# hellboywyh/pytorch-kaldi-CGS

Measured on AMD Instinct MI355X. Metric: acoustic frames/sec (train), higher is better.
Workload: dtype bf16; 1 GPU; TIMIT_baselines MLP 440-5x1024-{1928,48} (TIMIT_MLP_fmllr.cfg), batch_size_train=128, dropout 0.15, SGD body + RMSprop heads; global_batch=128, parallelism=dp1, chunk_frames_per_rank=225345

## Files before the change

### pytorch-kaldi-cgs_amd/csrc/pkc_fused.hip

```cpp
#include "pkc_common.h"

namespace pkc {
namespace fused {

constexpr int NW = 8, NT = 64 * NW;
constexpr int MR = 128;
constexpr int NC = 16;
constexpr int MT = MR / 16;

typedef __attribute__((ext_vector_type(8))) __bf16 bf8;
typedef __attribute__((ext_vector_type(4))) float f32x4;

#ifdef PKC_TRACE
constexpr int FTRACE_WG = 4096;
__device__ unsigned long long ftrace_buf[FTRACE_WG * 8];
__device__ __forceinline__ void ftrace(int i) {
  asm volatile("s_waitcnt vmcnt(0) lgkmcnt(0)" ::: "memory");
  const unsigned long long v = (i == 0 || i == 7) ? __builtin_amdgcn_s_memrealtime()
                                                  : __builtin_amdgcn_s_memtime();
  if (threadIdx.x == 0 && blockIdx.x < FTRACE_WG)
    reinterpret_cast<volatile unsigned long long*>(ftrace_buf)[blockIdx.x * 8 + i] = v;
}
#define PKC_FTR(i) ::pkc::fused::ftrace(i)
#else
#define PKC_FTR(i) do { } while (0)
#endif

__device__ __forceinline__ bf8 zero8() {
  bf8 v;
#pragma unroll
  for (int j = 0; j < 8; ++j) v[j] = (__bf16)0.f;
  return v;
}

template <bool BIN>
__device__ __forceinline__ bf8 ld8(const void* base, int64_t off) {
  if constexpr (BIN) {
    return *reinterpret_cast<const bf8*>(reinterpret_cast<const __bf16*>(base) + off);
  } else {
    const float* p = reinterpret_cast<const float*>(base) + off;
    const float4 x = *reinterpret_cast<const float4*>(p);
    const float4 y = *reinterpret_cast<const float4*>(p + 4);
    bf8 v;
    v[0] = (__bf16)x.x; v[1] = (__bf16)x.y; v[2] = (__bf16)x.z; v[3] = (__bf16)x.w;
    v[4] = (__bf16)y.x; v[5] = (__bf16)y.y; v[6] = (__bf16)y.z; v[7] = (__bf16)y.w;
    return v;
  }
}

constexpr int ROWS = MR + NC;
constexpr int IMG_BYTES = ROWS * 64;
constexpr int WAVE_BYTES = 2 * IMG_BYTES;
constexpr int STAGE_BYTES = NW * WAVE_BYTES;
constexpr int DMA_PER_STEP = ROWS * 4 / 64;

typedef __attribute__((address_space(3))) void lds_void;
typedef __attribute__((address_space(1))) const void glb_void;

__device__ __forceinline__ int img_h(int r) { return (-(r >> 2)) & 3; }

struct SlotSrc {
  int64_t off;
  bool isb;
  int k0;
};
__device__ __forceinline__ SlotSrc slot_src(int i, int lane, int ks, int M, int64_t lda, int64_t ldb,
                                            int n0) {
  const int r = 16 * i + (lane >> 2);
  const int kq = (lane & 3) ^ img_h(r);
  SlotSrc o;
  o.k0 = 32 * ks + 8 * kq;
  o.isb = r >= MR;
  o.off = o.isb ? (int64_t)(n0 + r - MR) * ldb + o.k0 : (int64_t)min(r, M - 1) * lda + o.k0;
  return o;
}

template <bool BIN>
__device__ __forceinline__ void stage_regs(char* img, const void* __restrict__ A, int64_t lda,
                                           const void* __restrict__ B, int64_t ldb, int M, int K,
                                           int n0, int ks) {
  const int lane = threadIdx.x & 63;
  const bf8 z8 = zero8();
  bf8 v[DMA_PER_STEP];
#pragma unroll
  for (int i = 0; i < DMA_PER_STEP; ++i) {
    const SlotSrc o = slot_src(i, lane, ks, M, lda, ldb, n0);
    const bool ok = o.k0 < K;
    const int64_t off = ok ? o.off : 0;
    const bf8 x = ld8<BIN>(o.isb ? B : A, off);
    v[i] = ok ? x : z8;
  }
#pragma unroll
  for (int i = 0; i < DMA_PER_STEP; ++i)
    *reinterpret_cast<bf8*>(img + 1024 * i + 16 * lane) = v[i];
}

__device__ __forceinline__ void stage_dma(char* img, const __bf16* __restrict__ A, int64_t lda,
                                          const __bf16* __restrict__ B, int64_t ldb, int M, int n0,
                                          int ks) {
  const int lane = threadIdx.x & 63;
#pragma unroll
  for (int i = 0; i < DMA_PER_STEP; ++i) {
    const SlotSrc o = slot_src(i, lane, ks, M, lda, ldb, n0);
    __builtin_amdgcn_global_load_lds((glb_void*)((o.isb ? B : A) + o.off),
                                     (lds_void*)(img + 1024 * i), 16, 0, 0);
  }
}

template <bool BIN>
__device__ __forceinline__ void strip_product(char* stage, const void* __restrict__ A, int64_t lda,
                                              const void* __restrict__ B, int64_t ldb, int M,
                                              int K, int n0, f32x4 (&acc)[MT]) {
  const int lane = threadIdx.x & 63;
  const int w = __builtin_amdgcn_readfirstlane(threadIdx.x >> 6);
  const int c = lane & 15, q = lane >> 4;
  const int nks = (K + 31) / 32;
  const int ks0 = w * nks / NW, ks1 = (w + 1) * nks / NW;
  const int nst = ks1 - ks0;
  char* mine = stage + w * WAVE_BYTES;
#pragma unroll
  for (int t = 0; t < MT; ++t) acc[t] = f32x4{0.f, 0.f, 0.f, 0.f};
  const int hq = (q ^ img_h(c)) * 16;
  const int afr = 64 * c + hq, bfr = 64 * (MR + c) + hq;
  const __bf16* Ab = reinterpret_cast<const __bf16*>(A);
  const __bf16* Bb = reinterpret_cast<const __bf16*>(B);
  auto issue = [&](int i) {
    char* img = mine + (i & 1) * IMG_BYTES;
    const int ks = ks0 + i;
    if (BIN && 32 * (ks + 1) <= K) stage_dma(img, Ab, lda, Bb, ldb, M, n0, ks);
    else stage_regs<BIN>(img, A, lda, B, ldb, M, K, n0, ks);
  };
  if (nst > 0) issue(0);
  if (nst > 1) issue(1);
  for (int i = 0; i < nst; ++i) {
    if (i + 1 < nst) asm volatile("s_waitcnt vmcnt(9)" ::: "memory");
    else asm volatile("s_waitcnt vmcnt(0)" ::: "memory");
    const char* img = mine + (i & 1) * IMG_BYTES;
    bf8 a[MT];
#pragma unroll
    for (int t = 0; t < MT; ++t) a[t] = *reinterpret_cast<const bf8*>(img + 1024 * t + afr);
    const bf8 b = *reinterpret_cast<const bf8*>(img + bfr);
    asm volatile("s_waitcnt lgkmcnt(0)" ::: "memory");
    if (i + 2 < nst) issue(i + 2);
#pragma unroll
    for (int t = 0; t < MT; ++t)
      acc[t] = __builtin_amdgcn_mfma_f32_16x16x32_bf16(a[t], b, acc[t], 0, 0, 0);
  }
}

__device__ __forceinline__ float4 strip_reduce(const f32x4 (&acc)[MT], float* red) {
  const int lane = threadIdx.x & 63, w = threadIdx.x >> 6;
  const int c = lane & 15, q = lane >> 4;
  float* mine = red + w * MR * NC;
#pragma unroll
  for (int t = 0; t < MT; ++t)
#pragma unroll
    for (int i = 0; i < 4; ++i) mine[(16 * t + 4 * q + i) * NC + c] = acc[t][i];
  __syncthreads();
  const int row = threadIdx.x >> 2, cg = threadIdx.x & 3;
  float4 z = *reinterpret_cast<const float4*>(red + row * NC + 4 * cg);
#pragma unroll
  for (int v = 1; v < NW; ++v) {
    const float4 p = *reinterpret_cast<const float4*>(red + v * MR * NC + row * NC + 4 * cg);
    z.x += p.x; z.y += p.y; z.z += p.z; z.w += p.w;
  }
  return z;
}

__device__ __forceinline__ float4 col_sum(float4 v, float4* xr) {
#pragma unroll
  for (int o = 4; o < 64; o <<= 1) {
    v.x += __shfl_xor(v.x, o, 64);
    v.y += __shfl_xor(v.y, o, 64);
    v.z += __shfl_xor(v.z, o, 64);
    v.w += __shfl_xor(v.w, o, 64);
  }
  const int lane = threadIdx.x & 63, w = threadIdx.x >> 6, cg = threadIdx.x & 3;
  if (lane < 4) xr[w * 4 + lane] = v;
  __syncthreads();
  float4 s = xr[cg];
#pragma unroll
  for (int u = 1; u < NW; ++u) {
    const float4 p = xr[u * 4 + cg];
    s.x += p.x; s.y += p.y; s.z += p.z; s.w += p.w;
  }
  return s;
}

__device__ __forceinline__ float f4g(const float4& v, int j) {
  return j == 0 ? v.x : (j == 1 ? v.y : (j == 2 ? v.z : v.w));
}
__device__ __forceinline__ void f4s(float4& v, int j, float x) {
  if (j == 0) v.x = x; else if (j == 1) v.y = x; else if (j == 2) v.z = x; else v.w = x;
}
__device__ __forceinline__ void st_h4(void* p, int64_t i, float4 v) {
  typedef __attribute__((ext_vector_type(4))) __bf16 bf16x4;
  bf16x4 h;
  h[0] = (__bf16)v.x; h[1] = (__bf16)v.y; h[2] = (__bf16)v.z; h[3] = (__bf16)v.w;
  *reinterpret_cast<bf16x4*>(reinterpret_cast<__bf16*>(p) + i) = h;
}

template <bool BIN>
__global__ __launch_bounds__(NT) void dense_gemm_fwd_kernel(const void* __restrict__ A, int64_t lda,
                                                           const void* __restrict__ W, int64_t ldw,
                                                           int K, pkc_dense_fwd_args a) {
  __shared__ __attribute__((aligned(16))) char stage[STAGE_BYTES];
  __shared__ float4 xr[2][NW * 4];
  float* red = reinterpret_cast<float*>(stage);
  static_assert(NW * MR * NC * 4 <= STAGE_BYTES, "partial strips must fit the staging LDS");
  PKC_FTR(0);
  const int n0 = blockIdx.x * NC;
  const int M = a.M;
  const int64_t N = a.N;
  const int row = threadIdx.x >> 2, cg = threadIdx.x & 3;
  const int c = n0 + 4 * cg;
  const float* dummy = a.gamma ? a.gamma : a.bias;
  const bool hb = a.bias != nullptr, bnp = a.norm != PKC_NORM_NONE && dummy != nullptr;
  const float* pd = dummy ? dummy : reinterpret_cast<const float*>(a.save_mean);
  const float4 b0 = *reinterpret_cast<const float4*>(hb ? a.bias + c : pd);
  const float4 g0 = *reinterpret_cast<const float4*>(bnp ? a.gamma + c : pd);
  const float4 be0 = *reinterpret_cast<const float4*>(bnp ? a.beta + c : pd);
  const float4 rm0 = *reinterpret_cast<const float4*>(bnp ? a.running_mean + c : pd);
  const float4 rv0 = *reinterpret_cast<const float4*>(bnp ? a.running_var + c : pd);
  const int64_t step = a.step_ctr ? *a.step_ctr : 0;
  PKC_FTR(1);
  f32x4 acc[MT];
  strip_product<BIN>(stage, A, lda, W, ldw, M, K, n0, acc);
  __syncthreads();
  PKC_FTR(2);
  float4 z = strip_reduce(acc, red);
  PKC_FTR(3);
  const bool rok = row < M;
  if (hb) z = make_float4(z.x + b0.x, z.y + b0.y, z.z + b0.z, z.w + b0.w);
  if (!rok) z = make_float4(0.f, 0.f, 0.f, 0.f);
  float4 mean = make_float4(0.f, 0.f, 0.f, 0.f), invstd = make_float4(1.f, 1.f, 1.f, 1.f);
  float4 gam = make_float4(1.f, 1.f, 1.f, 1.f), bet = make_float4(0.f, 0.f, 0.f, 0.f);
  if (a.norm == PKC_NORM_BN_TRAIN) {
    const float4 sum = col_sum(z, xr[0]);
    const float inv = 1.f / (float)M;
    mean = make_float4(sum.x * inv, sum.y * inv, sum.z * inv, sum.w * inv);
    float4 d2 = make_float4(0.f, 0.f, 0.f, 0.f);
    if (rok) {
      const float dx = z.x - mean.x, dy = z.y - mean.y, dz = z.z - mean.z, dw = z.w - mean.w;
      d2 = make_float4(dx * dx, dy * dy, dz * dz, dw * dw);
    }
    const float4 m2 = col_sum(d2, xr[1]);
    const float4 var = make_float4(m2.x * inv, m2.y * inv, m2.z * inv, m2.w * inv);
    invstd = make_float4(1.f / sqrtf(var.x + a.eps), 1.f / sqrtf(var.y + a.eps),
                         1.f / sqrtf(var.z + a.eps), 1.f / sqrtf(var.w + a.eps));
    gam = g0;
    bet = be0;
    if (row == 0) {
      *reinterpret_cast<float4*>(a.save_mean + c) = mean;
      *reinterpret_cast<float4*>(a.save_invstd + c) = invstd;
      const float cn = (float)(a.count_n > 0 ? a.count_n : M);
      float4 rm = rm0, rv = rv0;
#pragma unroll
      for (int j = 0; j < 4; ++j) {
        const float vj = f4g(var, j);
        const float unb = cn > 1.f ? vj * cn / (cn - 1.f) : vj;
        f4s(rm, j, (1.f - a.momentum) * f4g(rm, j) + a.momentum * f4g(mean, j));
        f4s(rv, j, (1.f - a.momentum) * f4g(rv, j) + a.momentum * unb);
      }
      *reinterpret_cast<float4*>(a.running_mean + c) = rm;
      *reinterpret_cast<float4*>(a.running_var + c) = rv;
    }
    PKC_FTR(4);
  } else if (a.norm == PKC_NORM_BN_EVAL) {
    mean = rm0;
    invstd = make_float4(1.f / sqrtf(rv0.x + a.eps), 1.f / sqrtf(rv0.y + a.eps),
                         1.f / sqrtf(rv0.z + a.eps), 1.f / sqrtf(rv0.w + a.eps));
    gam = g0;
    bet = be0;
  }
  if (!rok) return;
  const bool drop = a.drop_p > 0.f;
  const float scale = drop ? 1.f / (1.f - a.drop_p) : 1.f;
  const uint32_t thr = drop ? (uint32_t)((double)(1.f - a.drop_p) * 4294967296.0) : 0u;
  const uint32_t seed32 = hash_seed(a.seed, (uint64_t)a.stream_id, (uint64_t)step);
  const int64_t idx = (int64_t)row * N + c;
  float4 xh, o;
  uint32_t kw = 0;
  uchar4 kin = make_uchar4(1, 1, 1, 1);
  if (drop && a.keep_in) kin = *reinterpret_cast<const uchar4*>(a.keep_in + idx);
#pragma unroll
  for (int j = 0; j < 4; ++j) {
    const float zj = f4g(z, j);
    const float x = (a.norm == PKC_NORM_NONE) ? zj : (zj - f4g(mean, j)) * f4g(invstd, j);
    const float y = (a.norm == PKC_NORM_NONE) ? zj : x * f4g(gam, j) + f4g(bet, j);
    float v = act_fwd(a.act, y);
    if (drop) {
      uint32_t k;
      if (a.keep_in) k = j == 0 ? kin.x : (j == 1 ? kin.y : (j == 2 ? kin.z : kin.w));
      else k = hash_drop(seed32, (uint32_t)(idx + j)) < thr;
      kw |= (k ? 1u : 0u) << (8 * j);
      v = k ? v * scale : 0.f;
    }
    f4s(xh, j, x);
    f4s(o, j, v);
  }
  if (drop && a.keep_out) *reinterpret_cast<uint32_t*>(a.keep_out + idx) = kw;
  if (a.xhat) *reinterpret_cast<float4*>(a.xhat + idx) = xh;
  if (a.out) *reinterpret_cast<float4*>(a.out + idx) = o;
  if (a.out_bf16) st_h4(a.out_bf16, idx, o);
  PKC_FTR(5);
  PKC_FTR(7);
}

}
}

#ifdef PKC_TRACE
extern "C" int pkc_trace_read_fused(unsigned long long* host, int n) {
  return hipMemcpyFromSymbol(host, HIP_SYMBOL(pkc::fused::ftrace_buf), sizeof(unsigned long long) * n,
                             0, hipMemcpyDeviceToHost) == hipSuccess ? 0 : -1;
}
#endif

static bool al16(const void* p) { return (uintptr_t)p % 16 == 0; }

extern "C" int pkc_dense_gemm_fwd_ok(int prec, int M, int N, int K, const void* A, int64_t lda,
                                     const void* W, int64_t ldw) {
  using namespace pkc::fused;
  return (prec == PKC_PREC_BF16 || prec == PKC_PREC_BF16IN) && M > 0 && M <= MR && N > 0 &&
         N % NC == 0 && K > 0 && K % 8 == 0 && lda >= K && ldw >= K && lda % 8 == 0 &&
         ldw % 8 == 0 && al16(A) && al16(W) && lda < (1ll << 30) && ldw < (1ll << 30);
}

extern "C" int pkc_dense_gemm_fwd(int prec, const void* A, int64_t lda, const void* W, int64_t ldw,
                                  int K, const pkc_dense_fwd_args* a, void* stream) {
  using namespace pkc;
  using namespace pkc::fused;
  PKC_CHECK_ARG(a && A && W, "pkc_dense_gemm_fwd: null argument");
  PKC_CHECK_ARG(pkc_dense_gemm_fwd_ok(prec, a->M, a->N, K, A, lda, W, ldw),
                "pkc_dense_gemm_fwd: unsupported shape / precision / alignment (prec %d, M %d, "
                "N %d, K %d, lda %lld, ldw %lld)", prec, a->M, a->N, K, (long long)lda,
                (long long)ldw);
  PKC_CHECK_ARG(a->norm == PKC_NORM_NONE || a->norm == PKC_NORM_BN_TRAIN ||
                    a->norm == PKC_NORM_BN_EVAL,
                "pkc_dense_gemm_fwd: norm %d", a->norm);
  PKC_CHECK_ARG(a->norm == PKC_NORM_NONE || (a->gamma && a->beta && a->running_mean &&
                                             a->running_var),
                "pkc_dense_gemm_fwd: BatchNorm parameters missing");
  PKC_CHECK_ARG(a->norm != PKC_NORM_BN_TRAIN || (a->save_mean && a->save_invstd),
                "pkc_dense_gemm_fwd: BatchNorm training needs save_mean / save_invstd");
  PKC_CHECK_ARG(a->out || a->out_bf16, "pkc_dense_gemm_fwd: no output");
  PKC_CHECK_ARG((!a->out || al16(a->out)) && (!a->xhat || al16(a->xhat)) &&
                    (!a->out_bf16 || (uintptr_t)a->out_bf16 % 8 == 0) &&
                    (!a->bias || al16(a->bias)) && (!a->gamma || al16(a->gamma)) &&
                    (!a->beta || al16(a->beta)) && (!a->running_mean || al16(a->running_mean)) &&
                    (!a->running_var || al16(a->running_var)) &&
                    (!a->save_mean || al16(a->save_mean)) && (!a->save_invstd || al16(a->save_invstd)) &&
                    (!a->keep_out || (uintptr_t)a->keep_out % 4 == 0) &&
                    (!a->keep_in || (uintptr_t)a->keep_in % 4 == 0),
                "pkc_dense_gemm_fwd: outputs / parameters must be 16-byte aligned");
  PKC_CHECK_ARG(a->drop_p <= 0.f || a->keep_out || a->keep_in,
                "pkc_dense_gemm_fwd: dropout needs keep_out (or keep_in)");
  const dim3 grid(a->N / NC);
  if (prec == PKC_PREC_BF16IN)
    hipLaunchKernelGGL(dense_gemm_fwd_kernel<true>, grid, dim3(NT), 0, S(stream), A, lda, W, ldw, K,
                       *a);
  else
    hipLaunchKernelGGL(dense_gemm_fwd_kernel<false>, grid, dim3(NT), 0, S(stream), A, lda, W, ldw,
                       K, *a);
  PKC_LAUNCH_CHECK("pkc_dense_gemm_fwd");
  return PKC_OK;
}
```

Before: 928,600 frames/s.

## Split fused dense GEMM waves over row halves and K quarters with 64-wide k-steps

The strip-product work split changes. Before, all 8 waves split K eight ways. Now waves split into 2 row halves times 4 K-quarters, and each k-step covers 64 elements of K instead of 32. A new XOR swizzle and a reordered reduction row mapping come with this. The aim is to cut per-wave B-tile reloads and the cross-wave reduction cost (4 partials instead of 8), and to double the MFMA work issued per LDS wait. The reduction exchange buffers now live in the staging LDS, which shrinks the shared-memory footprint. The trace instrumentation also gains a K filter and realtime stamps, but that code only builds under PKC_TRACE.

```diff
diff --git a/pytorch-kaldi-cgs_amd/csrc/pkc_fused.hip b/pytorch-kaldi-cgs_amd/csrc/pkc_fused.hip
--- a/pytorch-kaldi-cgs_amd/csrc/pkc_fused.hip
+++ b/pytorch-kaldi-cgs_amd/csrc/pkc_fused.hip
@@ -6,7 +6,9 @@
 constexpr int NW = 8, NT = 64 * NW;
 constexpr int MR = 128;
 constexpr int NC = 16;
-constexpr int MT = MR / 16;
+constexpr int NKQ = 4, NRH = NW / NKQ;
+constexpr int RH = MR / NRH;
+constexpr int MT = RH / 16;
 
 typedef __attribute__((ext_vector_type(8))) __bf16 bf8;
 typedef __attribute__((ext_vector_type(4))) float f32x4;
@@ -14,14 +16,19 @@
 #ifdef PKC_TRACE
 constexpr int FTRACE_WG = 4096;
 __device__ unsigned long long ftrace_buf[FTRACE_WG * 8];
-__device__ __forceinline__ void ftrace(int i) {
+__device__ unsigned long long ftrace_rt[FTRACE_WG * 8];
+__device__ int ftrace_sel_k;
+__device__ __forceinline__ void ftrace(int i, int K) {
   asm volatile("s_waitcnt vmcnt(0) lgkmcnt(0)" ::: "memory");
-  const unsigned long long v = (i == 0 || i == 7) ? __builtin_amdgcn_s_memrealtime()
-                                                  : __builtin_amdgcn_s_memtime();
-  if (threadIdx.x == 0 && blockIdx.x < FTRACE_WG)
+  const unsigned long long rt = __builtin_amdgcn_s_memrealtime();
+  const unsigned long long v = (i == 0 || i == 7) ? rt : __builtin_amdgcn_s_memtime();
+  const int sel = *reinterpret_cast<volatile int*>(&ftrace_sel_k);
+  if (threadIdx.x == 0 && blockIdx.x < FTRACE_WG && (sel == 0 || sel == K)) {
     reinterpret_cast<volatile unsigned long long*>(ftrace_buf)[blockIdx.x * 8 + i] = v;
-}
-#define PKC_FTR(i) ::pkc::fused::ftrace(i)
+    reinterpret_cast<volatile unsigned long long*>(ftrace_rt)[blockIdx.x * 8 + i] = rt;
+  }
+}
+#define PKC_FTR(i) ::pkc::fused::ftrace(i, K)
 #else
 #define PKC_FTR(i) do { } while (0)
 #endif
@@ -48,43 +55,45 @@
   }
 }
 
-constexpr int ROWS = MR + NC;
-constexpr int IMG_BYTES = ROWS * 64;
+constexpr int KS = 64;
+constexpr int ROWS = RH + NC;
+constexpr int IMG_BYTES = ROWS * 2 * KS;
 constexpr int WAVE_BYTES = 2 * IMG_BYTES;
 constexpr int STAGE_BYTES = NW * WAVE_BYTES;
-constexpr int DMA_PER_STEP = ROWS * 4 / 64;
+constexpr int DMA_PER_STEP = ROWS * 8 / 64;
 
 typedef __attribute__((address_space(3))) void lds_void;
 typedef __attribute__((address_space(1))) const void glb_void;
 
-__device__ __forceinline__ int img_h(int r) { return (-(r >> 2)) & 3; }
+__device__ __forceinline__ int img_h(int r) { return (r >> 1) & 7; }
 
 struct SlotSrc {
   int64_t off;
   bool isb;
   int k0;
 };
-__device__ __forceinline__ SlotSrc slot_src(int i, int lane, int ks, int M, int64_t lda, int64_t ldb,
-                                            int n0) {
-  const int r = 16 * i + (lane >> 2);
-  const int kq = (lane & 3) ^ img_h(r);
+__device__ __forceinline__ SlotSrc slot_src(int i, int lane, int ks, int r0, int M, int64_t lda,
+                                            int64_t ldb, int n0) {
+  const int r = 8 * i + (lane >> 3);
+  const int kc = (lane & 7) ^ img_h(r);
   SlotSrc o;
-  o.k0 = 32 * ks + 8 * kq;
-  o.isb = r >= MR;
-  o.off = o.isb ? (int64_t)(n0 + r - MR) * ldb + o.k0 : (int64_t)min(r, M - 1) * lda + o.k0;
+  o.k0 = KS * ks + 8 * kc;
+  o.isb = r >= RH;
+  o.off = o.isb ? (int64_t)(n0 + r - RH) * ldb + o.k0
+                : (int64_t)min(r0 + r, M - 1) * lda + o.k0;
   return o;
 }
 
 template <bool BIN>
 __device__ __forceinline__ void stage_regs(char* img, const void* __restrict__ A, int64_t lda,
                                            const void* __restrict__ B, int64_t ldb, int M, int K,
-                                           int n0, int ks) {
+                                           int n0, int r0, int ks) {
   const int lane = threadIdx.x & 63;
   const bf8 z8 = zero8();
   bf8 v[DMA_PER_STEP];
 #pragma unroll
   for (int i = 0; i < DMA_PER_STEP; ++i) {
-    const SlotSrc o = slot_src(i, lane, ks, M, lda, ldb, n0);
+    const SlotSrc o = slot_src(i, lane, ks, r0, M, lda, ldb, n0);
     const bool ok = o.k0 < K;
     const int64_t off = ok ? o.off : 0;
     const bf8 x = ld8<BIN>(o.isb ? B : A, off);
@@ -97,11 +106,11 @@
 
 __device__ __forceinline__ void stage_dma(char* img, const __bf16* __restrict__ A, int64_t lda,
                                           const __bf16* __restrict__ B, int64_t ldb, int M, int n0,
-                                          int ks) {
+                                          int r0, int ks) {
   const int lane = threadIdx.x & 63;
 #pragma unroll
   for (int i = 0; i < DMA_PER_STEP; ++i) {
-    const SlotSrc o = slot_src(i, lane, ks, M, lda, ldb, n0);
+    const SlotSrc o = slot_src(i, lane, ks, r0, M, lda, ldb, n0);
     __builtin_amdgcn_global_load_lds((glb_void*)((o.isb ? B : A) + o.off),
                                      (lds_void*)(img + 1024 * i), 16, 0, 0);
   }
@@ -114,53 +123,66 @@
   const int lane = threadIdx.x & 63;
   const int w = __builtin_amdgcn_readfirstlane(threadIdx.x >> 6);
   const int c = lane & 15, q = lane >> 4;
-  const int nks = (K + 31) / 32;
-  const int ks0 = w * nks / NW, ks1 = (w + 1) * nks / NW;
-  const int nst = ks1 - ks0;
+  const int r0 = RH * (w % NRH), kr = w / NRH;
+  const int nks = (K + KS - 1) / KS;
+  const int ks0 = kr * nks / NKQ, ks1 = (kr + 1) * nks / NKQ;
+  const int nst = r0 < M ? ks1 - ks0 : 0;
   char* mine = stage + w * WAVE_BYTES;
 #pragma unroll
   for (int t = 0; t < MT; ++t) acc[t] = f32x4{0.f, 0.f, 0.f, 0.f};
-  const int hq = (q ^ img_h(c)) * 16;
-  const int afr = 64 * c + hq, bfr = 64 * (MR + c) + hq;
+  const int h0 = (q ^ img_h(c)) * 16, h1 = ((4 + q) ^ img_h(c)) * 16;
+  const int afr = 128 * c, bfr = 128 * (RH + c);
   const __bf16* Ab = reinterpret_cast<const __bf16*>(A);
   const __bf16* Bb = reinterpret_cast<const __bf16*>(B);
   auto issue = [&](int i) {
     char* img = mine + (i & 1) * IMG_BYTES;
     const int ks = ks0 + i;
-    if (BIN && 32 * (ks + 1) <= K) stage_dma(img, Ab, lda, Bb, ldb, M, n0, ks);
-    else stage_regs<BIN>(img, A, lda, B, ldb, M, K, n0, ks);
+    if (BIN && KS * (ks + 1) <= K) stage_dma(img, Ab, lda, Bb, ldb, M, n0, r0, ks);
+    else stage_regs<BIN>(img, A, lda, B, ldb, M, K, n0, r0, ks);
   };
   if (nst > 0) issue(0);
   if (nst > 1) issue(1);
   for (int i = 0; i < nst; ++i) {
-    if (i + 1 < nst) asm volatile("s_waitcnt vmcnt(9)" ::: "memory");
+    if (i + 1 < nst) asm volatile("s_waitcnt vmcnt(10)" ::: "memory");
     else asm volatile("s_waitcnt vmcnt(0)" ::: "memory");
+    static_assert(DMA_PER_STEP == 10, "the counted wait above is one k-step's DMA instructions");
     const char* img = mine + (i & 1) * IMG_BYTES;
-    bf8 a[MT];
-#pragma unroll
-    for (int t = 0; t < MT; ++t) a[t] = *reinterpret_cast<const bf8*>(img + 1024 * t + afr);
-    const bf8 b = *reinterpret_cast<const bf8*>(img + bfr);
+    bf8 a0[MT], a1[MT];
+#pragma unroll
+    for (int t = 0; t < MT; ++t) {
+      a0[t] = *reinterpret_cast<const bf8*>(img + 2048 * t + afr + h0);
+      a1[t] = *reinterpret_cast<const bf8*>(img + 2048 * t + afr + h1);
+    }
+    const bf8 b0 = *reinterpret_cast<const bf8*>(img + bfr + h0);
+    const bf8 b1 = *reinterpret_cast<const bf8*>(img + bfr + h1);
     asm volatile("s_waitcnt lgkmcnt(0)" ::: "memory");
+    if (i == 0) PKC_FTR(6);
     if (i + 2 < nst) issue(i + 2);
 #pragma unroll
     for (int t = 0; t < MT; ++t)
-      acc[t] = __builtin_amdgcn_mfma_f32_16x16x32_bf16(a[t], b, acc[t], 0, 0, 0);
-  }
-}
+      acc[t] = __builtin_amdgcn_mfma_f32_16x16x32_bf16(a0[t], b0, acc[t], 0, 0, 0);
+#pragma unroll
+    for (int t = 0; t < MT; ++t)
+      acc[t] = __builtin_amdgcn_mfma_f32_16x16x32_bf16(a1[t], b1, acc[t], 0, 0, 0);
+  }
+}
+
+__device__ __forceinline__ int red_row(int r) { return (r & ~7) | ((r & 3) << 1) | ((r >> 2) & 1); }
 
 __device__ __forceinline__ float4 strip_reduce(const f32x4 (&acc)[MT], float* red) {
   const int lane = threadIdx.x & 63, w = threadIdx.x >> 6;
   const int c = lane & 15, q = lane >> 4;
-  float* mine = red + w * MR * NC;
+  float* mine = red + (w / NRH) * MR * NC;
+  const int r0 = RH * (w % NRH);
 #pragma unroll
   for (int t = 0; t < MT; ++t)
 #pragma unroll
-    for (int i = 0; i < 4; ++i) mine[(16 * t + 4 * q + i) * NC + c] = acc[t][i];
+    for (int i = 0; i < 4; ++i) mine[red_row(r0 + 16 * t + 4 * q + i) * NC + c] = acc[t][i];
   __syncthreads();
-  const int row = threadIdx.x >> 2, cg = threadIdx.x & 3;
+  const int row = red_row(threadIdx.x >> 2), cg = threadIdx.x & 3;
   float4 z = *reinterpret_cast<const float4*>(red + row * NC + 4 * cg);
 #pragma unroll
-  for (int v = 1; v < NW; ++v) {
+  for (int v = 1; v < NKQ; ++v) {
     const float4 p = *reinterpret_cast<const float4*>(red + v * MR * NC + row * NC + 4 * cg);
     z.x += p.x; z.y += p.y; z.z += p.z; z.w += p.w;
   }
@@ -205,9 +227,12 @@
                                                            const void* __restrict__ W, int64_t ldw,
                                                            int K, pkc_dense_fwd_args a) {
   __shared__ __attribute__((aligned(16))) char stage[STAGE_BYTES];
-  __shared__ float4 xr[2][NW * 4];
+  constexpr int RED_BYTES = NKQ * MR * NC * 4;
   float* red = reinterpret_cast<float*>(stage);
-  static_assert(NW * MR * NC * 4 <= STAGE_BYTES, "partial strips must fit the staging LDS");
+  float4* xr[2] = {reinterpret_cast<float4*>(stage + RED_BYTES),
+                   reinterpret_cast<float4*>(stage + RED_BYTES) + NW * 4};
+  static_assert(RED_BYTES + 2 * NW * 4 * 16 <= STAGE_BYTES,
+                "partial strips and exchanges must fit the staging LDS");
   PKC_FTR(0);
   const int n0 = blockIdx.x * NC;
   const int M = a.M;
@@ -315,6 +340,14 @@
   return hipMemcpyFromSymbol(host, HIP_SYMBOL(pkc::fused::ftrace_buf), sizeof(unsigned long long) * n,
                              0, hipMemcpyDeviceToHost) == hipSuccess ? 0 : -1;
 }
+extern "C" int pkc_trace_read_fused_rt(unsigned long long* host, int n) {
+  return hipMemcpyFromSymbol(host, HIP_SYMBOL(pkc::fused::ftrace_rt), sizeof(unsigned long long) * n,
+                             0, hipMemcpyDeviceToHost) == hipSuccess ? 0 : -1;
+}
+extern "C" int pkc_trace_fused_select(int K) {
+  return hipMemcpyToSymbol(HIP_SYMBOL(pkc::fused::ftrace_sel_k), &K, sizeof(int), 0,
+                           hipMemcpyHostToDevice) == hipSuccess ? 0 : -1;
+}
 #endif
 
 static bool al16(const void* p) { return (uintptr_t)p % 16 == 0; }
```

After: 929,900 frames/s (median of 3 runs). No clear change (+0.1%).
